# YukinoriMatsuoka/indy-plenum

Measured on AMD Instinct MI355X. Metric: Ed25519 verifies/sec at 1/8 MI355X (256B msgs) + % of INT32 VALU peak vs host CPU, higher is better.
Workload: dtype int32

## Files before the change

indy-plenum_amd/csrc/edv_hostcheck.cpp:

```cpp
#define EDV_CHAIN_FLOOR 1
#include <stdint.h>
#include <string.h>
#include <vector>
#include "edv_verify_core.h"
#include "edv_sha256.h"
#include "edv_merkle.h"
#include "edv_ledger.h"
#include "edv_tables.h"
#include "edv_hostplan.h"
#include "edv_selftest_cases.h"
#include "edv_probe_ops.h"

using namespace edv;

namespace {
struct HostATab {
  ge_cached t[kAEntries];
  int staged = 0;
  void store(int e, const ge_cached& c) { t[e] = c; }
  ge_cached load(int e) const { return t[e]; }
  void stage(int e) { staged = e; }
  ge_cached fetch() const { return t[staged]; }
};
struct HostBTab {
// ... 94 lines not shown
    const uint64_t mlen = off[i + 1] - off[i];
    std::vector<uint8_t> buf(mlen + 48, 0);
    if (mlen) memcpy(buf.data() + 16, msgs + off[i], mlen);
    uint32_t o[8];
    sha256_msg(o, buf.data() + 16, mlen);
    store_words(out + 32 * i, o, 8);
  }
  return 0;
}
int hc_btab_entries_of_bits(int bits, int t, const int32_t* js, int nj, int32_t* out) {
  if (bits != kBBits && bits != kBBitsCompact) return -1;
  const HostBTab& b = btab(bits);
  if (t < 0 || t >= b.sh.tables) return -1;
  for (int k = 0; k < nj; k++) {
    if (js[k] < 0 || js[k] >= b.sh.entries) return -1;
    btab_entry(out + size_t(k) * kBStride, js[k], b.base[t]);
  }
  return 0;
}
int hc_btab_entries_of(int t, const int32_t* js, int nj, int32_t* out) {
  return hc_btab_entries_of_bits(kBBits, t, js, nj, out);
}
int hc_rside_point_bits(int bits, const uint8_t* R32, const uint8_t* S32, uint8_t* out32) {
  struct Keep {
    ge_cached q;
    void store(int e, const ge_cached& c) { if (e == 1) q = c; }
  } tab;
  uint32_t R[8], S[8], o[8];
  load_words(R, R32, 8);
  load_words(S, S32, 8);
  if (bits != kBBits && bits != kBBitsCompact) return -1;
  HostBStage bs{btab(bits)};
  if (!prep_rpoint(R, S, tab, bs)) return -1;
  const fe two_y = fe_carry32(fe_add(tab.q.YpX, tab.q.YmX)), two_x = fe_carry32(fe_sub(tab.q.YpX, tab.q.YmX));
  ge_p2 p{two_x, two_y, fe_carry32(fe_add(tab.q.Z, tab.q.Z))};
  ge_p2_tobytes(o, p);
  store_words(out32, o, 8);
  return 0;
}
int hc_rside_point(const uint8_t* R32, const uint8_t* S32, uint8_t* out32) {
  return hc_rside_point_bits(kBBits, R32, S32, out32);
}
int hc_half_scalars(const uint8_t* h32, uint8_t* a32, uint8_t* u32) {
  uint32_t h[8], a[8], u[8];
  load_words(h, h32, 8);
  bool neg = false;
  half_scalars(h, a, u, neg);
  store_words(a32, a, 8);
  store_words(u32, u, 8);
  return neg ? 1 : 0;
}
int hc_probe_math(int op, const void* in, uint64_t in_stride, void* out, uint64_t out_stride, uint64_t n) {
  const ProbeSize sz = probe_size(op);
  if (!sz.in || probe_is_quad(op) || in_stride < sz.in || out_stride < sz.out || (in_stride & 3) || (out_stride & 3))
    return -1;
  for (uint64_t i = 0; i < n; i++) {
    const uint32_t* x = reinterpret_cast<const uint32_t*>(static_cast<const uint8_t*>(in) + i * in_stride);
    uint32_t* y = reinterpret_cast<uint32_t*>(static_cast<uint8_t*>(out) + i * out_stride);
    switch (op) {
#define HC_PROBE_CASE(OP) case OP: probe_lane_op<OP>(x, y); break;
      HC_PROBE_CASE(EDV_PROBE_FE_MUL)
      HC_PROBE_CASE(EDV_PROBE_FE_SQ)
      HC_PROBE_CASE(EDV_PROBE_FE_SQ2)
      HC_PROBE_CASE(EDV_PROBE_FE_SQ_FLOOR)
      HC_PROBE_CASE(EDV_PROBE_FE_TOBYTES)
      HC_PROBE_CASE(EDV_PROBE_FE_FROMBYTES)
      HC_PROBE_CASE(EDV_PROBE_FE_INVERT_SAFEGCD)
      HC_PROBE_CASE(EDV_PROBE_FE_POW22523)
      HC_PROBE_CASE(EDV_PROBE_SC_REDUCE)
      HC_PROBE_CASE(EDV_PROBE_HALF_SCALARS)
      HC_PROBE_CASE(EDV_PROBE_RECODE5)
      HC_PROBE_CASE(EDV_PROBE_APPROX_DIV)
      HC_PROBE_CASE(EDV_PROBE_FDIV_FLOOR)
      HC_PROBE_CASE(EDV_PROBE_EUCLID_DIV)
      HC_PROBE_CASE(EDV_PROBE_GE_FROMBYTES)
      HC_PROBE_CASE(EDV_PROBE_SC_MULADD)
      HC_PROBE_CASE(EDV_PROBE_RECODE8)
      HC_PROBE_CASE(EDV_PROBE_GE_P3_TOBYTES)
#undef HC_PROBE_CASE
      case EDV_PROBE_SCALARMULT_BASE: probe_scalarmult_base(x, y, comb()); break;
      default: return -1;
    }
  }
  return 0;
}
static_assert(kAEntries * 40 == 360, "a slot's table is 9 entries of 4 x 10 limbs");
int hc_stage_prep(const uint8_t* sigs, const uint8_t* pks, const uint8_t* msgs, const uint64_t* off, uint64_t n,
                  int bits, int side0, int nsides, int buckets, uint64_t cap, uint32_t* dig, uint8_t* alive,
                  int32_t* atab, int32_t* rtab, uint32_t* perm, uint8_t* accept) {
  if ((bits != kBBits && bits != kBBitsCompact) || n > cap || side0 < 0 || nsides < 1 || side0 + nsides > 3) return -1;
  const HostBTab& bt = btab(bits);
  if (buckets) {
    auto bucket = [&](uint64_t i) {
      const uint64_t nb = (64 + (off[i + 1] - off[i]) + 17 + 127) / 128;
      return nb < 63 ? nb : uint64_t(63);
    };
    uint64_t k = 0;
    bool one = true;
    for (uint64_t i = 1; i < n; i++) one = one && bucket(i) == bucket(0);
    for (uint64_t b = 0; b < 64 && !one; b++)
      for (uint64_t i = 0; i < n; i++)
        if (bucket(i) == b) perm[k++] = uint32_t(i);
    for (uint64_t i = 0; one && i < n; i++) perm[i] = uint32_t(i);
  }
  for (uint64_t j = 0; j < n; j++) {
    const uint64_t i = buckets ? perm[j] : j;
    uint32_t R[8], S[8], A[8];
    load_words(R, sigs + 64 * i, 8);
    load_words(S, sigs + 64 * i + 32, 8);
    load_words(A, pks + 32 * i, 8);
    for (int side = side0; side < side0 + nsides; side++) {
      bool ok;
      if (side == 0) {
        const uint64_t mlen = off[i + 1] - off[i];
        std::vector<uint8_t> buf(mlen + 32, 0);
        if (mlen) memcpy(buf.data() + 16, msgs + off[i], mlen);
        PrepDigits pd;
        ok = prep_one(R, S, A, buf.data() + 16, mlen, pd);
        if (ok) {
          for (int k = 0; k < 8; k++) {
            dig[uint64_t(k) * cap + j] = pd.da[k];
            dig[uint64_t(8 + k) * cap + j] = pd.db[k];
          }
          dig[16 * cap + j] = uint32_t(pd.nwin) | (pd.negR ? 0x100u : 0u);
        }
      } else {
        HostATab tab;
        if (side == 1) {
          ok = prep_point(A, tab);
        } else {
          HostBStage bs{bt};
          ok = prep_rpoint(R, S, tab, bs);
        }
        int32_t* o = (side == 1 ? atab : rtab) + j * 360;
        for (int e = 0; ok && e < kAEntries; e++) {
          from_fe(o + 40 * e, tab.t[e].YpX);
          from_fe(o + 40 * e + 10, tab.t[e].YmX);
          from_fe(o + 40 * e + 20, tab.t[e].Z);
          from_fe(o + 40 * e + 30, tab.t[e].T2d);
        }
      }
      alive[uint64_t(side) * cap + j] = ok ? 1 : 0;
      if (!ok) accept[i] = 0;
    }
  }
  return 0;
}
int hc_stage_main(uint64_t n, uint64_t cap, const uint32_t* dig, const uint8_t* alive, const int32_t* atab,
                  const int32_t* rtab, const uint32_t* perm, uint8_t* accept) {
  if (n > cap) return -1;
  auto live = [&](uint64_t j) { return j < n && alive[j] && alive[cap + j] && alive[2 * cap + j]; };
  for (uint64_t w0 = 0; w0 < n; w0 += 64) {
    int nwin = 0;
    for (uint64_t j = w0; j < w0 + 64; j++)
      if (live(j)) nwin = mx(nwin, int(dig[16 * cap + j] & 0xff));
    if (nwin > kAWindows) return -1;
    for (uint64_t j = w0; j < w0 + 64; j++) {
      if (!live(j)) continue;
      if (perm && perm[j] >= n) return -1;
      uint32_t da[8], db[8];
      for (int k = 0; k < 8; k++) {
        da[k] = dig[uint64_t(k) * cap + j];
        db[k] = dig[uint64_t(8 + k) * cap + j];
      }
      HostATab at, rt;
      for (int e = 0; e < kAEntries; e++) {
        const int32_t *a = atab + j * 360 + 40 * e, *r = rtab + j * 360 + 40 * e;
        at.t[e] = ge_cached{to_fe(a), to_fe(a + 10), to_fe(a + 20), to_fe(a + 30)};
        rt.t[e] = ge_cached{to_fe(r), to_fe(r + 10), to_fe(r + 20), to_fe(r + 30)};
      }
      accept[perm ? perm[j] : j] = main_one(da, db, nwin, (dig[16 * cap + j] >> 8) & 1, at, rt) ? 1 : 0;
    }
  }
  return 0;
}
namespace {
void put_p3(int32_t* pt, int k, uint64_t slots, uint64_t j, const ge_p3& p) {
  const fe* c[4] = {&p.X, &p.Y, &p.Z, &p.T};
  for (int q = 0; q < 4; q++)
    for (int i = 0; i < 10; i++) pt[(uint64_t(k) * 40 + 10 * q + i) * slots + j] = c[q]->v[i];
}
ge_p3 get_p3(const int32_t* pt, int k, uint64_t slots, uint64_t j) {
  fe c[4];
  for (int q = 0; q < 4; q++)
    for (int i = 0; i < 10; i++) c[q].v[i] = pt[(uint64_t(k) * 40 + 10 * q + i) * slots + j];
  return ge_p3{c[0], c[1], c[2], c[3]};
}
ge_p3 p3_add(const ge_p3& p, const ge_p3& q) { return ge_p1p1_to_p3(ge_add(p, ge_p3_to_cached(q))); }
ge_p3 p3_neg(const ge_p3& p) { return ge_p3{fe_neg(p.X), p.Y, p.Z, fe_neg(p.T)}; }
ge_p3 signed_digit_mult(const uint32_t d[8], bool negate, const ge_p3& P) {
  ge_p3 m[9];
  m[0] = ge_p3_identity();
  for (int e = 1; e < 9; e++) m[e] = p3_add(m[e - 1], P);
  ge_p3 acc = ge_p3_identity();
  for (int k = 63; k >= 0; k--) {
    for (int t = 0; t < 4; t++) acc = ge_p1p1_to_p3(ge_p2_dbl(ge_p3_to_p2(acc)));
    int dg = int(d[k / 8] >> (4 * (k % 8))) & 15;
    if (dg >= 8) dg -= 16;
    if (negate) dg = -dg;
    if (dg) acc = p3_add(acc, dg < 0 ? p3_neg(m[-dg]) : m[dg]);
  }
  return acc;
}
}
int hc_stage_latency_phase1(const uint8_t* sigs, const uint8_t* pks, const uint8_t* msgs, const uint64_t* off,
                            uint64_t n, int ns, int bits, uint32_t* dig, int32_t* pt, uint8_t* ok) {
  if ((bits != kBBits && bits != kBBitsCompact) || (ns != 16 && ns != 32) || n == 0) return -1;
  const HostBTab& bt = btab(bits);
  const uint64_t slots = (n + ns - 1) / ns * ns;
  for (uint64_t jl = 0; jl < slots; jl++) {
    const bool in = jl < n || jl < 16;
    const uint64_t i = jl < n ? jl : n - 1;
    bool ok0 = false, ok1 = false, ok2 = false;
    PrepDigits pd;
    ge_p3 pa = ge_p3_identity(), pr = ge_p3_identity(), sb = ge_p3_identity();
    if (in) {
      uint32_t R[8], S[8], A[8];
      load_words(R, sigs + 64 * i, 8);
      load_words(S, sigs + 64 * i + 32, 8);
      load_words(A, pks + 32 * i, 8);
      const uint64_t mlen = off[i + 1] - off[i];
      std::vector<uint8_t> buf(mlen + 32, 0);
      if (mlen) memcpy(buf.data() + 16, msgs + off[i], mlen);
      ok0 = prep_one(R, S, A, buf.data() + 16, mlen, pd);
      ok1 = ge_is_canonical(A) && !has_small_order(A) && ge_frombytes_negate(pa, A);
      if (!ok1) pa = ge_p3_identity();
      ok2 = ge_is_canonical(R) && !has_small_order(R) && ge_frombytes_negate(pr, R);
      if (!ok2) pr = ge_p3_identity();
      HostBStage bs{bt};
      add_sb(sb, S, bs);
    }
    for (int k = 0; k < 8; k++) {
      dig[uint64_t(k) * slots + jl] = ok0 ? pd.da[k] : 0u;
      dig[uint64_t(8 + k) * slots + jl] = ok0 ? pd.db[k] : 0u;
    }
    dig[16 * slots + jl] = ok0 ? (uint32_t(pd.nwin) | (pd.negR ? 0x100u : 0u)) : 0u;
    ok[jl] = ok0;
    ok[slots + jl] = ok1;
    ok[2 * slots + jl] = ok2;
    put_p3(pt, 0, slots, jl, pa);
    put_p3(pt, 1, slots, jl, pr);
    put_p3(pt, 2, slots, jl, sb);
  }
  return 0;
}
int hc_stage_latency_walk(uint64_t n, int ns, const uint32_t* dig, const int32_t* pt, const uint8_t* ok,
                          uint8_t* accept) {
  if ((ns != 16 && ns != 32) || n == 0) return -1;
  const uint64_t slots = (n + ns - 1) / ns * ns;
  for (uint64_t j = 0; j < n; j++) {
    const bool alive = ok[j] && ok[slots + j] && ok[2 * slots + j];
    if (!alive) {
      accept[j] = 0;
      continue;
    }
    const uint32_t wf = dig[16 * slots + j];
    if ((wf & 0xff) > uint32_t(kAWindows)) return -1;
    uint32_t da[8], db[8];
    for (int k = 0; k < 8; k++) {
      da[k] = dig[uint64_t(k) * slots + j];
      db[k] = dig[uint64_t(8 + k) * slots + j];
    }
    const ge_p3 q = p3_add(get_p3(pt, 2, slots, j), get_p3(pt, 1, slots, j));
    const ge_p3 r = p3_add(signed_digit_mult(da, false, get_p3(pt, 0, slots, j)),
                           signed_digit_mult(db, (wf >> 8) & 1, q));
    accept[j] = (fe_iszero(r.X) && fe_iszero(fe_sub(r.Y, r.Z))) ? 1 : 0;
  }
  return 0;
}
int hc_comb_entries(const int32_t* ij, int n, int32_t* out) {
  const HostComb& ct = comb();
  for (int k = 0; k < n; k++) {
    if (ij[2 * k] < 0 || ij[2 * k] >= kCombRows || ij[2 * k + 1] < 0 || ij[2 * k + 1] >= kCombEntries) return -1;
    memcpy(out + size_t(k) * kBStride, ct.w.data() + (ij[2 * k] * kCombEntries + ij[2 * k + 1]) * kBStride,
           kBStride * sizeof(int32_t));
  }
  return 0;
}
double hc_approx_div(double a, double b) { return approx_div(a, b); }
double hc_fdiv_floor(double a, double b) { return fdiv_floor(a, b); }
void hc_euclid_div(uint32_t* r0, uint32_t* t0, const uint32_t* r1, const uint32_t* t1) { euclid_div(r0, t0, r1, t1); }
int hc_recode5_windows(const uint8_t* in32, uint32_t* out8) {
  uint32_t w[8];
  load_words(w, in32, 8);
  recode5(out8, w);
  return digits5_windows(out8);
}
int hc_ge_frombytes_negate_limbs(const uint8_t* in32, int32_t* out40) {
  uint32_t w[8];
  load_words(w, in32, 8);
  ge_p3 p;
  const bool ok = ge_frombytes_negate(p, w);
  from_fe(out40, p.X);
  from_fe(out40 + 10, p.Y);
  from_fe(out40 + 20, p.Z);
  from_fe(out40 + 30, p.T);
  return int(ge_is_canonical(w)) | int(has_small_order(w)) << 1 | int(ok) << 2;
}
void hc_ge_add_p3(const int32_t* p40, const int32_t* q40, int32_t* out40) {
  const ge_p3 p{to_fe(p40), to_fe(p40 + 10), to_fe(p40 + 20), to_fe(p40 + 30)};
  const ge_p3 q{to_fe(q40), to_fe(q40 + 10), to_fe(q40 + 20), to_fe(q40 + 30)};
  const ge_p3 r = ge_p1p1_to_p3(ge_add(p, ge_p3_to_cached(q)));
  from_fe(out40, r.X); from_fe(out40 + 10, r.Y); from_fe(out40 + 20, r.Z); from_fe(out40 + 30, r.T);
}
void hc_ge_dbl_p3(const int32_t* p40, int32_t* out40) {
  const ge_p3 p{to_fe(p40), to_fe(p40 + 10), to_fe(p40 + 20), to_fe(p40 + 30)};
  const ge_p3 r = ge_p1p1_to_p3(ge_p2_dbl(ge_p3_to_p2(p)));
  from_fe(out40, r.X); from_fe(out40 + 10, r.Y); from_fe(out40 + 20, r.Z); from_fe(out40 + 30, r.T);
}
void hc_layout(int32_t* out4) {
  const int32_t v[4] = {kAWin, kAEntries, kBBits, kBTables};
  memcpy(out4, v, sizeof v);
}
int hc_btab_entries() { return kBEntries; }
void hc_ledger(int64_t n, const int64_t* failed, int nf, const int64_t* queries, int nq, int* out) {
  AsyncLedger l;
  for (int64_t i = 0; i < n; i++) l.issue();
  for (int k = 0; k < nf; k++) l.fail(failed[k]);
  for (int k = 0; k < nq; k++) out[k] = l.settled(queries[k]);
}
void hc_choose_tables(int policy, uint64_t n, int have_compact, int have_large, int failed, int* out3) {
  const TableChoice c = choose_tables(policy, n, have_compact != 0, have_large != 0, failed != 0);
  out3[0] = c.use;
  out3[1] = c.build;
  out3[2] = c.failed ? 1 : 0;
}
void hc_packed_layout(uint64_t n, uint64_t mbytes, uint64_t* out5) {
// ... 317 lines not shown
```

indy-plenum_amd/csrc/edv_verify.hip:

```cpp
#include <hip/hip_runtime.h>
#include <stdint.h>

#include "edv_verify_core.h"
#include "edv_kernels.h"
#include "edv_launch.h"
#include "edv_sha256.h"

using namespace edv;

namespace {

constexpr int kEntryPieces = 10;
constexpr int kLdsAWords = kEntryPieces * 256;
constexpr int kLdsWaveWords = 2 * kLdsAWords;
__device__ __forceinline__ void wait_staged() { asm volatile("s_waitcnt vmcnt(0)" ::: "memory"); }
struct LdsATab {
  const int32_t* slot;
  int32_t* lds;
  int lane;
  __device__ __forceinline__ void stage(int e) {
    const int32_t* g = slot + e * kEntryWords;
#pragma unroll
    for (int q = 0; q < kEntryPieces; q++)
      __builtin_amdgcn_global_load_lds(const_cast<int32_t*>(g + 4 * q), lds + q * 256, 16, 0, 0);
  }
  __device__ __forceinline__ ge_cached fetch() {
    wait_staged();
    int32_t t[4 * kEntryPieces];
#pragma unroll
    for (int q = 0; q < kEntryPieces; q++) {
      const int4 v = reinterpret_cast<const int4*>(lds + q * 256)[lane];
      t[4 * q] = v.x; t[4 * q + 1] = v.y; t[4 * q + 2] = v.z; t[4 * q + 3] = v.w;
    }
    ge_cached c;
#pragma unroll
    for (int l = 0; l < 10; l++) {
      c.YpX.v[l] = t[l]; c.YmX.v[l] = t[10 + l]; c.Z.v[l] = t[20 + l]; c.T2d.v[l] = t[30 + l];
    }
    return c;
  }
};
#define EDV_MAIN_BODY \
  const uint64_t j = uint64_t(blockIdx.x) * kBlock + threadIdx.x; \
  const bool live = j < a.n && a.st.alive[j] && a.st.alive[a.st.cap + j] && a.st.alive[2 * a.st.cap + j]; \
  const uint32_t* d = a.st.dig + j; \
  const uint64_t cap = a.st.cap; \
  const uint32_t wf = live ? d[uint64_t(kDigNwin) * cap] : 0; \
  int nwin = int(wf & 0xff); \
_Pragma("unroll") \
  for (int o = 32; o > 0; o >>= 1) nwin = max(nwin, __shfl_xor(nwin, o)); \
  nwin = __builtin_amdgcn_readfirstlane(nwin); \
  if (!live) return; \
  const uint64_t i = a.base + (a.st.perm ? a.st.perm[j] : j); \
  uint32_t da[8], db[8]; \
_Pragma("unroll") \
  for (int k = 0; k < 8; k++) { \
    da[k] = d[uint64_t(k) * cap]; \
    db[k] = d[uint64_t(8 + k) * cap]; \
  } \
_Pragma("unroll") \
  for (int k = 0; k < 8; k++) { \
    da[k] = uint32_t(opaque_i32(int32_t(da[k]))); \
    db[k] = uint32_t(opaque_i32(int32_t(db[k]))); \
  } \
  int32_t* wl = lds_main + (threadIdx.x >> 6) * kLdsWaveWords; \
  const int lane = int(threadIdx.x & 63); \
  LdsATab at{a.st.atab + j * kAWords, wl, lane}, rt{a.st.rtab + j * kAWords, wl + kLdsAWords, lane}; \
  a.accept[i] = main_one(da, db, nwin, (wf >> 8) & 1, at, rt) ? 1 : 0;

__global__ __launch_bounds__(kBlock) void edv_main_kernel(VerifyArgs a) {
  __shared__ int32_t lds_main[(kBlock / 64) * kLdsWaveWords];
  EDV_MAIN_BODY
}

constexpr int kSplitMainPrio = 2;
__global__ __launch_bounds__(kBlock) void edv_main_kernel_prio(VerifyArgs a) {
  __shared__ int32_t lds_main[(kBlock / 64) * kLdsWaveWords];
  __builtin_amdgcn_s_setprio(kSplitMainPrio);
  EDV_MAIN_BODY
}

__global__ __launch_bounds__(kBlock) void edv_sign_kernel(const uint32_t* seeds, const uint8_t* msgs,
                                                          const uint64_t* off, uint64_t msg_base, uint64_t n,
                                                          uint32_t* pks, uint32_t* sigs, const int32_t* comb) {
  const uint64_t i = uint64_t(blockIdx.x) * kBlock + threadIdx.x;
  if (i >= n) return;
  uint32_t seed[8], pk[8], sig[16];
  load_words(seed, seeds + 8 * i, 2);
  const uint64_t o0 = off[i] - msg_base, o1 = off[i + 1] - msg_base;
  sign_one(pk, sig, seed, msgs + o0, o1 - o0, GlobalComb{comb});
  uint4* po = reinterpret_cast<uint4*>(pks + 8 * i);
  uint4* so = reinterpret_cast<uint4*>(sigs + 16 * i);
  po[0] = make_uint4(pk[0], pk[1], pk[2], pk[3]);
  po[1] = make_uint4(pk[4], pk[5], pk[6], pk[7]);
#pragma unroll
  for (int k = 0; k < 4; k++) so[k] = make_uint4(sig[4 * k], sig[4 * k + 1], sig[4 * k + 2], sig[4 * k + 3]);
}

__global__ void edv_comb_kernel(int32_t* out) {
  const int t = threadIdx.x + blockIdx.x * blockDim.x;
  if (t < kCombRows * kCombEntries) comb_entry(out + t * kBStride, t / kCombEntries, t % kCombEntries);
}

__device__ __forceinline__ uint32_t sha_bucket(const uint64_t* off, uint64_t i) {
  const uint64_t nb = (64 + (off[i + 1] - off[i]) + 17 + 127) / 128;
  return nb < kBuckets - 1 ? uint32_t(nb) : uint32_t(kBuckets - 1);
}
__global__ __launch_bounds__(kBlock) void edv_bucket_hist_kernel(const uint64_t* off, uint64_t base, uint64_t n,
                                                                 uint32_t* hist) {
  __shared__ uint32_t h[kBuckets];
  if (threadIdx.x < kBuckets) h[threadIdx.x] = 0;
  __syncthreads();
  const uint64_t j = uint64_t(blockIdx.x) * kBlock + threadIdx.x;
  if (j < n) atomicAdd(&h[sha_bucket(off, base + j)], 1u);
  __syncthreads();
  if (threadIdx.x < kBuckets && h[threadIdx.x]) atomicAdd(&hist[threadIdx.x], h[threadIdx.x]);
}
__global__ __launch_bounds__(kBlock) void edv_bucket_scatter_kernel(const uint64_t* off, uint64_t base, uint64_t n,
                                                                    const uint32_t* hist, uint32_t* cursor,
                                                                    uint32_t* perm) {
  __shared__ uint32_t start[kBuckets], cnt[kBuckets], wbase[kBuckets];
  __shared__ int nonempty;
  if (threadIdx.x == 0) {
    uint32_t acc = 0;
    int ne = 0;
    for (int b = 0; b < kBuckets; b++) { start[b] = acc; acc += hist[b]; ne += hist[b] != 0; }
    nonempty = ne;
  }
  if (threadIdx.x < kBuckets) cnt[threadIdx.x] = 0;
  __syncthreads();
  const uint64_t j = uint64_t(blockIdx.x) * kBlock + threadIdx.x;
  if (nonempty <= 1) {
    if (j < n) perm[j] = uint32_t(j);
    return;
  }
  uint32_t b = 0, rank = 0;
  if (j < n) {
    b = sha_bucket(off, base + j);
    rank = atomicAdd(&cnt[b], 1u);
  }
  __syncthreads();
  if (threadIdx.x < kBuckets && cnt[threadIdx.x])
    wbase[threadIdx.x] = start[threadIdx.x] + atomicAdd(&cursor[threadIdx.x], cnt[threadIdx.x]);
  __syncthreads();
  if (j < n) perm[wbase[b] + rank] = uint32_t(j);
}

__global__ __launch_bounds__(kBlock) void edv_pack_bits_kernel(const uint8_t* acc, uint64_t n, uint8_t* bits) {
  const uint64_t k = uint64_t(blockIdx.x) * kBlock + threadIdx.x;
  if (8 * k >= n) return;
  uint32_t b = 0;
  if (8 * k + 8 <= n && !(reinterpret_cast<uintptr_t>(acc) & 3)) {
    const uint32_t lo = reinterpret_cast<const uint32_t*>(acc)[2 * k], hi = reinterpret_cast<const uint32_t*>(acc)[2 * k + 1];
#pragma unroll
    for (int t = 0; t < 4; t++) b |= (((lo >> (8 * t)) & 0xff) != 0 ? 1u : 0u) << t;
#pragma unroll
    for (int t = 0; t < 4; t++) b |= (((hi >> (8 * t)) & 0xff) != 0 ? 1u : 0u) << (4 + t);
  } else {
    for (uint64_t i = 8 * k; i < n && i < 8 * k + 8; i++) b |= (acc[i] != 0 ? 1u : 0u) << (i - 8 * k);
  }
  bits[k] = uint8_t(b);
}

__global__ void edv_bbase_kernel(ge_p3* bases, SbShape sh) {
  if (int(threadIdx.x) < sh.tables) bases[threadIdx.x] = base_point(int(threadIdx.x) * sh.bits);
}
__global__ void edv_btab_kernel(int32_t* out, const ge_p3* bases, SbShape sh) {
  const uint32_t t = threadIdx.x + blockIdx.x * blockDim.x;
  if (t < uint32_t(sh.tables * sh.entries))
    btab_entry(out + size_t(t) * kBStride, int(t % uint32_t(sh.entries)), bases[t / uint32_t(sh.entries)]);
}

__global__ __launch_bounds__(kBlock) void edv_sha256_kernel(const uint8_t* msgs, const uint64_t* off, uint64_t msg_base,
                                                            uint64_t n, uint32_t* out) {
  const uint64_t i = uint64_t(blockIdx.x) * kBlock + threadIdx.x;
  if (i >= n) return;
  const uint64_t o0 = off[i] - msg_base, o1 = off[i + 1] - msg_base;
  uint32_t d[8];
  sha256_msg(d, msgs + o0, o1 - o0);
  uint4* po = reinterpret_cast<uint4*>(out + 8 * i);
  po[0] = make_uint4(d[0], d[1], d[2], d[3]);
  po[1] = make_uint4(d[4], d[5], d[6], d[7]);
}

}

namespace edv {

hipError_t launch_main_kernel(unsigned blocks, hipStream_t s, const VerifyArgs& va, bool prio) {
  if (prio) edv_main_kernel_prio<<<dim3(blocks), dim3(kBlock), 0, s>>>(va);
  else edv_main_kernel<<<dim3(blocks), dim3(kBlock), 0, s>>>(va);
  return hipGetLastError();
}
hipError_t launch_bucket_kernels(unsigned blocks, hipStream_t s, const uint64_t* off, uint64_t base, uint64_t n,
                                 uint32_t* ctr, uint32_t* perm) {
  edv_bucket_hist_kernel<<<dim3(blocks), dim3(kBlock), 0, s>>>(off, base, n, ctr);
  edv_bucket_scatter_kernel<<<dim3(blocks), dim3(kBlock), 0, s>>>(off, base, n, ctr, ctr + kBuckets, perm);
  return hipGetLastError();
}
hipError_t launch_btab_kernel(hipStream_t s, int32_t* out, SbShape sh) {
  ge_p3* bases = reinterpret_cast<ge_p3*>(out + sb_words(sh));
  edv_bbase_kernel<<<1, 64, 0, s>>>(bases, sh);
  edv_btab_kernel<<<(sh.tables * sh.entries + 63) / 64, 64, 0, s>>>(out, bases, sh);
  return hipGetLastError();
}
hipError_t launch_comb_kernel(hipStream_t s, int32_t* out) {
  edv_comb_kernel<<<(kCombRows * kCombEntries + 63) / 64, 64, 0, s>>>(out);
  return hipGetLastError();
}
hipError_t launch_sign_kernel(unsigned blocks, hipStream_t s, const uint32_t* seeds, const uint8_t* msgs,
                              const uint64_t* off, uint64_t msg_base, uint64_t n, uint32_t* pks, uint32_t* sigs,
                              const int32_t* comb) {
  edv_sign_kernel<<<dim3(blocks), dim3(kBlock), 0, s>>>(seeds, msgs, off, msg_base, n, pks, sigs, comb);
  return hipGetLastError();
}
hipError_t launch_pack_bits_kernel(hipStream_t s, const uint8_t* acc, uint64_t n, uint8_t* bits) {
  const uint64_t nb = (n + 7) / 8;
  edv_pack_bits_kernel<<<dim3(unsigned((nb + kBlock - 1) / kBlock)), dim3(kBlock), 0, s>>>(acc, n, bits);
  return hipGetLastError();
}
hipError_t launch_sha256_kernel(unsigned blocks, hipStream_t s, const uint8_t* msgs, const uint64_t* off,
// ... 7 lines not shown
```

indy-plenum_amd/csrc/edv_verify_core.h:

```cpp
#pragma once
#include "edv_math.h"

namespace edv {

constexpr int kAWin = 4;
constexpr int kAWindows = (255 + kAWin - 1) / kAWin;
constexpr int kAEntries = (1 << (kAWin - 1)) + 1;
constexpr int kBBits = 22;
constexpr int kBTables = (253 + kBBits - 1) / kBBits;
constexpr int kBEntries = (1 << (kBBits - 1)) + 1;
constexpr int kBBitsCompact = 16;
constexpr int kBTablesCompact = (253 + kBBitsCompact - 1) / kBBitsCompact;
constexpr int kBEntriesCompact = (1 << (kBBitsCompact - 1)) + 1;
static_assert(253 - kBBits * (kBTables - 1) <= kBBits - 1, "top [S]B digit out of table range");
static_assert(253 - kBBitsCompact * (kBTablesCompact - 1) <= kBBitsCompact - 1, "top [S]B digit out of table range");
struct SbShape {
  int bits, tables, entries;
};
EDV_HD constexpr SbShape sb_large() { return SbShape{kBBits, kBTables, kBEntries}; }
EDV_HD constexpr SbShape sb_compact() { return SbShape{kBBitsCompact, kBTablesCompact, kBEntriesCompact}; }
constexpr int kCombEntries = 129;
constexpr int kBStride = 32;

EDV_HD int mx(int a, int b) { return a > b ? a : b; }
// ... 403 lines not shown
#pragma unroll
  for (int i = 0; i < 7; i++) v[i] = (v[i] >> N) | (v[i + 1] << (32 - N));
  v[7] >>= N;
}

EDV_HD ge_precomp precomp_from_words(const int32_t* w) {
  ge_precomp q;
#pragma unroll
  for (int l = 0; l < 10; l++) { q.ypx.v[l] = w[l]; q.ymx.v[l] = w[10 + l]; q.xy2d.v[l] = w[20 + l]; }
  return q;
}

EDV_HD ge_p3 base_point(int shift) {
  const uint32_t Bw[8] = {0x66666658u, 0x66666666u, 0x66666666u, 0x66666666u,
                          0x66666666u, 0x66666666u, 0x66666666u, 0x66666666u};
  ge_p3 nB;
  ge_frombytes_negate(nB, Bw);
  ge_p3 B{fe_neg(nB.X), nB.Y, nB.Z, fe_neg(nB.T)};
  for (int k = 0; k < shift; k++) B = ge_p1p1_to_p3(ge_p2_dbl(ge_p3_to_p2(B)));
  return B;
}
EDV_HD void btab_entry(int32_t* o, int j, const ge_p3& base) {
  const ge_cached Bc = ge_p3_to_cached(base);
  ge_p3 acc = ge_p3_identity();
  for (int bit = kBBits - 1; bit >= 0; bit--) {
    acc = ge_p1p1_to_p3(ge_p2_dbl(ge_p3_to_p2(acc)));
    if ((j >> bit) & 1) acc = ge_p1p1_to_p3(ge_add(acc, Bc));
  }
  const fe zi = fe_invert(acc.Z);
  const fe x = fe_mul(acc.X, zi), y = fe_mul(acc.Y, zi);
  const fe ypx = fe_carry32(fe_add(y, x)), ymx = fe_carry32(fe_sub(y, x));
  const fe xy2d = fe_mul(fe_mul(x, y), fe_d2());
  for (int l = 0; l < 10; l++) { o[l] = ypx.v[l]; o[10 + l] = ymx.v[l]; o[20 + l] = xy2d.v[l]; }
  o[30] = 0;
  o[31] = 0;
}

EDV_HD constexpr size_t sb_words(SbShape sh) { return size_t(sh.tables) * size_t(sh.entries) * kBStride; }
EDV_HD constexpr size_t sb_alloc_bytes(SbShape sh) { return 4 * sb_words(sh) + size_t(sh.tables) * sizeof(ge_p3); }

struct PrepDigits {
  uint32_t da[8];
  uint32_t db[8];
  int nwin;
  bool negR;
};

template <class Tab>
EDV_HD void build_table(Tab& tab, const ge_p3& P) {
  const ge_cached c1 = ge_p3_to_cached(P);
  const ge_precomp p1{c1.YpX, c1.YmX, c1.T2d};
  tab.store(0, ge_cached_identity());
  tab.store(1, c1);
  ge_p3 cur = ge_p1p1_to_p3(ge_p2_dbl(ge_p3_to_p2(P)));
  tab.store(2, ge_p3_to_cached(cur));
#pragma unroll 1
  for (int e = 3; e < kAEntries; e++) {
    cur = ge_p1p1_to_p3(ge_madd(cur, p1));
    tab.store(e, ge_p3_to_cached(cur));
  }
}
template <class Tab, class Stash>
EDV_HD void build_table_projective(Tab& tab, const ge_p3& P, Stash& st) {
  {
    const ge_cached c1 = ge_p3_to_cached(P);
    tab.store(0, ge_cached_identity());
    tab.store(1, c1);
    st.put(c1);
  }
  ge_p3 cur = ge_p1p1_to_p3(ge_p2_dbl(ge_p3_to_p2(P)));
  tab.store(2, ge_p3_to_cached(cur));
#pragma unroll 1
  for (int e = 3; e < kAEntries; e++) {
    cur = ge_p1p1_to_p3(ge_add(cur, st.get()));
    tab.store(e, ge_p3_to_cached(cur));
  }
}

EDV_HD bool prep_one(const uint32_t R[8], const uint32_t S[8], const uint32_t A[8], const uint8_t* m, uint64_t mlen,
                     PrepDigits& pd) {
  bool ok = !((S[7] & 0xF0000000u) && !sc_is_canonical(S));
  ok = ok && !has_small_order(R);
  ok = ok && ge_is_canonical(A) && !has_small_order(A);
  if (!ok) return false;
  uint32_t dig[16], h[8];
  hram(dig, R, A, m, mlen);
  sc_reduce(h, dig);
  uint32_t a[8], u[8];
  bool neg;
  half_scalars(h, a, u, neg);
  recode5(pd.da, a);
  recode5(pd.db, u);
  pd.nwin = mx(digits5_windows(pd.da), digits5_windows(pd.db));
  pd.negR = neg;
  return true;
}

template <class ATab>
EDV_HD bool prep_point(const uint32_t P[8], ATab& tab) {
  if (!ge_is_canonical(P) || has_small_order(P)) return false;
  ge_p3 nP;
  if (!ge_frombytes_negate(nP, P)) return false;
  build_table(tab, nP);
  return true;
}

EDV_HD void shr256_var(uint32_t v[8], int n) {
#pragma unroll
  for (int i = 0; i < 7; i++) v[i] = (v[i] >> n) | (v[i + 1] << (32 - n));
  v[7] >>= n;
}
template <class BTab>
EDV_HD void add_sb(ge_p3& q, const uint32_t S[8], BTab& bt) {
  const SbShape sh = bt.shape();
  uint32_t s[8];
#pragma unroll
  for (int i = 0; i < 8; i++) s[i] = S[i];
  s[7] &= 0x1fffffffu;
  int carry = 0;
  const int bits = sh.bits;
  auto next_digit = [&](bool top) {
    int e = int(s[0] & ((1u << bits) - 1)) + carry;
    shr256_var(s, bits);
    carry = top ? 0 : (e + (1 << (bits - 1))) >> bits;
    return e - carry * (1 << bits);
  };
  int dt = next_digit(sh.tables == 1);
  bt.stage(0, dt < 0 ? -dt : dt);
#pragma unroll 1
  for (int t = 0; t < sh.tables; t++) {
    const ge_precomp e = ge_precomp_cneg(bt.fetch(), dt < 0);
    if (t + 1 < sh.tables) {
      dt = next_digit(t + 2 == sh.tables);
      bt.stage(t + 1, dt < 0 ? -dt : dt);
    }
    q = ge_p1p1_to_p3(ge_madd(q, e));
  }
}
template <class BTab>
EDV_HD bool rpoint_q(const uint32_t R[8], const uint32_t S[8], BTab& bt, ge_p3& q) {
  if (!ge_is_canonical(R) || has_small_order(R)) return false;
  if (!ge_frombytes_negate(q, R)) return false;
  add_sb(q, S, bt);
  return true;
}
template <class ATab, class BTab>
EDV_HD bool prep_rpoint(const uint32_t R[8], const uint32_t S[8], ATab& tab, BTab& bt) {
  ge_p3 q;
  if (!rpoint_q(R, S, bt, q)) return false;
  build_table_projective(tab, q, bt);
  return true;
}

template <class ATab>
EDV_HD bool main_one(uint32_t da[8], uint32_t db[8], int nwin, bool negR, ATab& at, ATab& rt) {
  constexpr int kTop = kAWin * (kAWindows - 1);
  constexpr int kTopShl = 32 - kAWin - (kTop - 224);
#pragma unroll 1
  for (int k = nwin; k < kAWindows; k++) {
    shl256<kAWin>(da);
    shl256<kAWin>(db);
  }
  ge_p2 acc = ge_p2_identity();
#pragma unroll 1
  for (int w = nwin - 1; w >= 0; --w) {
    const int dA = int32_t(da[7] << kTopShl) >> (32 - kAWin);
    const int dR = int32_t(db[7] << kTopShl) >> (32 - kAWin);
    shl256<kAWin>(da);
    shl256<kAWin>(db);
    at.stage(dA < 0 ? -dA : dA);
    rt.stage(dR < 0 ? -dR : dR);
    ge_p3 p3;
    if (w == nwin - 1) {
      p3 = ge_p3_identity();
    } else {
#pragma unroll 1
      for (int d = 0; d < kAWin - 1; d++) acc = ge_p1p1_to_p2(ge_p2_dbl(acc));
      p3 = ge_p1p1_to_p3(ge_p2_dbl(acc));
    }
    const ge_cached ea = at.fetch();
    p3 = ge_p1p1_to_p3(ge_add(p3, ge_cached_cneg(ea, dA < 0)));
    const ge_cached er = rt.fetch();
    acc = ge_p1p1_to_p2(ge_add(p3, ge_cached_cneg(er, (dR < 0) != negR)));
  }
  return fe_iszero(acc.X) && fe_iszero(fe_carry32(fe_sub(acc.Y, acc.Z)));
}

template <class ATab, class BTab>
EDV_HD bool verify_one(const uint32_t R[8], const uint32_t S[8], const uint32_t A[8], const uint8_t* m, uint64_t mlen,
                       ATab& at, ATab& rt, BTab& bt) {
  PrepDigits pd;
  if (!prep_one(R, S, A, m, mlen, pd)) return false;
  if (!prep_point(A, at) || !prep_rpoint(R, S, rt, bt)) return false;
  return main_one(pd.da, pd.db, pd.nwin, pd.negR, at, rt);
}

constexpr int kCombRows = 32;
EDV_HD void comb_entry(int32_t* o, int i, int j) {
  const uint32_t Bw[8] = {0x66666658u, 0x66666666u, 0x66666666u, 0x66666666u,
                          0x66666666u, 0x66666666u, 0x66666666u, 0x66666666u};
  ge_p3 nB;
  ge_frombytes_negate(nB, Bw);
  ge_p3 base{fe_neg(nB.X), nB.Y, nB.Z, fe_neg(nB.T)};
  for (int k = 0; k < 8 * i; k++) base = ge_p1p1_to_p3(ge_p2_dbl(ge_p3_to_p2(base)));
  const ge_cached bc = ge_p3_to_cached(base);
  ge_p3 acc = ge_p3_identity();
  for (int bit = 7; bit >= 0; bit--) {
    acc = ge_p1p1_to_p3(ge_p2_dbl(ge_p3_to_p2(acc)));
    if ((j >> bit) & 1) acc = ge_p1p1_to_p3(ge_add(acc, bc));
  }
  const fe zi = fe_invert(acc.Z);
  const fe x = fe_mul(acc.X, zi), y = fe_mul(acc.Y, zi);
  const fe ypx = fe_carry32(fe_add(y, x)), ymx = fe_carry32(fe_sub(y, x));
  const fe xy2d = fe_mul(fe_mul(x, y), fe_d2());
  for (int l = 0; l < 10; l++) { o[l] = ypx.v[l]; o[10 + l] = ymx.v[l]; o[20 + l] = xy2d.v[l]; }
  o[30] = 0;
  o[31] = 0;
}
template <class CombTab>
EDV_HD ge_p3 scalarmult_base(const uint32_t k[8], const CombTab& ct) {
  uint32_t d[8];
  recode8(d, k);
  ge_p3 acc = ge_p3_identity();
#pragma unroll 1
  for (int i = 0; i < kCombRows; i++) {
    const int di = int(int8_t(uint8_t(d[i >> 2] >> (8 * (i & 3)))));
    const int ui = di < 0 ? -di : di;
    acc = ge_p1p1_to_p3(ge_madd(acc, ge_precomp_cneg(ct.entry(i, ui), di < 0)));
  }
  return acc;
}
EDV_HD void ge_p3_tobytes(uint32_t w[8], const ge_p3& p) { ge_p2_tobytes(w, ge_p3_to_p2(p)); }

EDV_HD void sc_muladd(uint32_t out[8], const uint32_t a[8], const uint32_t b[8], const uint32_t c[8]) {
  uint32_t t[16];
  uint64_t carry = 0;
#pragma unroll
  for (int k = 0; k < 16; k++) {
    uint64_t lo = carry + (k < 8 ? c[k] : 0), hi = 0;
#pragma unroll
    for (int i = 0; i < 8; i++) {
      const int j = k - i;
      if (j < 0 || j > 7) continue;
      const uint64_t p = uint64_t(a[i]) * b[j];
      const uint64_t s = lo + p;
      hi += (s < lo);
      lo = s;
    }
    t[k] = uint32_t(lo);
    carry = (lo >> 32) | (hi << 32);
  }
  sc_reduce(out, t);
}

template <class CombTab>
EDV_HD void sign_one(uint32_t pk[8], uint32_t sig[16], const uint32_t seed[8], const uint8_t* m, uint64_t mlen,
                     const CombTab& ct) {
  uint32_t az[16];
  sha512_pm<32>(az, seed, m, 0);
  az[0] &= ~7u;
  az[7] = (az[7] & 0x7fffffffu) | 0x40000000u;
  uint32_t a64[16], a[8];
#pragma unroll
  for (int k = 0; k < 16; k++) a64[k] = k < 8 ? az[k] : 0;
  sc_reduce(a, a64);
  ge_p3_tobytes(pk, scalarmult_base(a, ct));
  uint32_t nonce[16], r[8];
  sha512_pm<32>(nonce, az + 8, m, mlen);
  sc_reduce(r, nonce);
  ge_p3_tobytes(sig, scalarmult_base(r, ct));
  uint32_t hr[16], h[8];
  hram(hr, sig, pk, m, mlen);
  sc_reduce(h, hr);
  uint32_t aclamped[8];
#pragma unroll
  for (int k = 0; k < 8; k++) aclamped[k] = az[k];
  sc_muladd(sig + 8, h, aclamped, r);
}

}
```

Measured before the change: 97.80 million.

## Fold small top window digit into table-entry additions to skip four doublings

When the wave's top window index is 34 and every lane's top digit is small (0..2), the top window is folded away. It is replaced by up to two additions of table entry 8 (which equals 8P) before the next window, so 16·e·P is handled as 2·(e·8P). That removes one window's four doublings at the cost of up to four extra point additions and wave-wide ballots. Host check paths and test helpers are extended to mirror the new recoding.

After: 97.98 million (median of 6 runs). No clear change (+0.2%).

```diff
diff --git a/indy-plenum_amd/csrc/edv_hostcheck.cpp b/indy-plenum_amd/csrc/edv_hostcheck.cpp
--- a/indy-plenum_amd/csrc/edv_hostcheck.cpp
+++ b/indy-plenum_amd/csrc/edv_hostcheck.cpp
@@ -270,9 +270,16 @@
   auto live = [&](uint64_t j) { return j < n && alive[j] && alive[cap + j] && alive[2 * cap + j]; };
   for (uint64_t w0 = 0; w0 < n; w0 += 64) {
     int nwin = 0;
-    for (uint64_t j = w0; j < w0 + 64; j++)
-      if (live(j)) nwin = mx(nwin, int(dig[16 * cap + j] & 0xff));
+    uint32_t max_e = 0;
+    for (uint64_t j = w0; j < w0 + 64; j++) {
+      if (!live(j)) continue;
+      const uint32_t ea = (dig[uint64_t(kWideWord) * cap + j] >> kWideShift) & 15u;
+      const uint32_t eb = (dig[uint64_t(8 + kWideWord) * cap + j] >> kWideShift) & 15u;
+      nwin = mx(nwin, wide_fold_count(int(dig[16 * cap + j] & 0xff), ea, eb));
+      max_e = (ea | eb) & 2u ? 2u : (max_e ? max_e : ((ea | eb) ? 1u : 0u));
+    }
     if (nwin > kAWindows) return -1;
+    const int wide = wide_rounds(nwin, max_e);
     for (uint64_t j = w0; j < w0 + 64; j++) {
       if (!live(j)) continue;
       if (perm && perm[j] >= n) return -1;
@@ -287,10 +294,62 @@
         at.t[e] = ge_cached{to_fe(a), to_fe(a + 10), to_fe(a + 20), to_fe(a + 30)};
         rt.t[e] = ge_cached{to_fe(r), to_fe(r + 10), to_fe(r + 20), to_fe(r + 30)};
       }
-      accept[perm ? perm[j] : j] = main_one(da, db, nwin, (dig[16 * cap + j] >> 8) & 1, at, rt) ? 1 : 0;
+      accept[perm ? perm[j] : j] =
+          main_one(da, db, nwin, (dig[16 * cap + j] >> 8) & 1, at, rt, wide, wide_digit(da), wide_digit(db)) ? 1 : 0;
     }
   }
   return 0;
+}
+void hc_wide_recode(const uint8_t* in32, uint32_t* out8, int32_t* out3) {
+  uint32_t w[8];
+  load_words(w, in32, 8);
+  recode5(out8, w);
+  const int own = digits5_windows(out8);
+  const uint32_t e = wide_digit(out8);
+  const int nwin = wide_fold_count(own, e, 0);
+  out3[0] = nwin;
+  out3[1] = own;
+  out3[2] = nwin < own ? int32_t(e) : 0;
+  if (nwin < own) out8[kWideWord] &= ~(15u << kWideShift);
+}
+void hc_wide_lane(const uint8_t* a32, const uint8_t* u32, int32_t* out4) {
+  uint32_t a[8], u[8], da[8], db[8];
+  load_words(a, a32, 8);
+  load_words(u, u32, 8);
+  recode5(da, a);
+  recode5(db, u);
+  const int own = mx(digits5_windows(da), digits5_windows(db));
+  const int nwin = wide_fold_count(own, wide_digit(da), wide_digit(db));
+  out4[0] = own;
+  out4[1] = nwin;
+  out4[2] = nwin < own ? int32_t(wide_digit(da)) : 0;
+  out4[3] = nwin < own ? int32_t(wide_digit(db)) : 0;
+}
+int hc_main_one(const uint8_t* a32, const uint8_t* u32, int negR, const int32_t* p1_40, const int32_t* p2_40,
+                int wave_nwin, int wide) {
+  uint32_t a[8], u[8], da[8], db[8];
+  load_words(a, a32, 8);
+  load_words(u, u32, 8);
+  recode5(da, a);
+  recode5(db, u);
+  const uint32_t ea = wide_digit(da), eb = wide_digit(db);
+  const int own = wide_fold_count(mx(digits5_windows(da), digits5_windows(db)), ea, eb);
+  const int nwin = wave_nwin ? wave_nwin : own;
+  const uint32_t me = ea > eb ? ea : eb;
+  if (nwin < own || nwin > kAWindows) return -1;
+  if (wide < 0) wide = wide_rounds(nwin, me);
+  if (wide < wide_rounds(nwin, me) || (wide && (nwin != kWideWin || wide > int(kWideMaxE)))) return -1;
+  HostATab at, rt;
+  const ge_p3 p1{to_fe(p1_40), to_fe(p1_40 + 10), to_fe(p1_40 + 20), to_fe(p1_40 + 30)};
+  const ge_p3 p2{to_fe(p2_40), to_fe(p2_40 + 10), to_fe(p2_40 + 20), to_fe(p2_40 + 30)};
+  struct NoStash {
+    ge_cached c;
+    void put(const ge_cached& x) { c = x; }
+    ge_cached get() const { return c; }
+  } st;
+  build_table_projective(at, p1, st);
+  build_table_projective(rt, p2, st);
+  return main_one(da, db, nwin, negR != 0, at, rt, wide, ea, eb) ? 1 : 0;
 }
 namespace {
 void put_p3(int32_t* pt, int k, uint64_t slots, uint64_t j, const ge_p3& p) {
diff --git a/indy-plenum_amd/csrc/edv_verify.hip b/indy-plenum_amd/csrc/edv_verify.hip
--- a/indy-plenum_amd/csrc/edv_verify.hip
+++ b/indy-plenum_amd/csrc/edv_verify.hip
@@ -46,10 +46,13 @@
   const uint32_t* d = a.st.dig + j; \
   const uint64_t cap = a.st.cap; \
   const uint32_t wf = live ? d[uint64_t(kDigNwin) * cap] : 0; \
-  int nwin = int(wf & 0xff); \
+  const uint32_t ea = live ? (d[uint64_t(kWideWord) * cap] >> kWideShift) & 15u : 0; \
+  const uint32_t eb = live ? (d[uint64_t(8 + kWideWord) * cap] >> kWideShift) & 15u : 0; \
+  int nwin = wide_fold_count(int(wf & 0xff), ea, eb); \
 _Pragma("unroll") \
   for (int o = 32; o > 0; o >>= 1) nwin = max(nwin, __shfl_xor(nwin, o)); \
   nwin = __builtin_amdgcn_readfirstlane(nwin); \
+  const int wide = wide_rounds(nwin, __ballot(((ea | eb) & 2u) != 0) ? 2u : (__ballot((ea | eb) != 0) ? 1u : 0u)); \
   if (!live) return; \
   const uint64_t i = a.base + (a.st.perm ? a.st.perm[j] : j); \
   uint32_t da[8], db[8]; \
@@ -66,7 +69,7 @@
   int32_t* wl = lds_main + (threadIdx.x >> 6) * kLdsWaveWords; \
   const int lane = int(threadIdx.x & 63); \
   LdsATab at{a.st.atab + j * kAWords, wl, lane}, rt{a.st.rtab + j * kAWords, wl + kLdsAWords, lane}; \
-  a.accept[i] = main_one(da, db, nwin, (wf >> 8) & 1, at, rt) ? 1 : 0;
+  a.accept[i] = main_one(da, db, nwin, (wf >> 8) & 1, at, rt, wide, ea, eb) ? 1 : 0;
 
 __global__ __launch_bounds__(kBlock) void edv_main_kernel(VerifyArgs a) {
   __shared__ int32_t lds_main[(kBlock / 64) * kLdsWaveWords];
diff --git a/indy-plenum_amd/csrc/edv_verify_core.h b/indy-plenum_amd/csrc/edv_verify_core.h
--- a/indy-plenum_amd/csrc/edv_verify_core.h
+++ b/indy-plenum_amd/csrc/edv_verify_core.h
@@ -579,16 +579,61 @@
   return true;
 }
 
+constexpr int kWideWin = 33;
+constexpr uint32_t kWideMaxE = 2;
+static_assert(kAWin == 4, "the wide top is laid out for 4-bit windows: 16 e P = 2 (e x entry 8)");
+constexpr int kWideWord = (4 * kWideWin) >> 5, kWideShift = (4 * kWideWin) & 31;
+EDV_HD uint32_t wide_digit(const uint32_t d[8]) { return (d[kWideWord] >> kWideShift) & 15u; }
+EDV_HD int wide_fold_count(int nwin, uint32_t ea, uint32_t eb) {
+  static_assert(kWideMaxE == 2, "the range test below is e + 1 < 4");
+  const uint32_t out = nz_mask(uint32_t(nwin) ^ uint32_t(kWideWin + 1)) | nz_mask(((ea + 1) | (eb + 1)) >> 2);
+  return nwin - int(~out & 1u);
+}
+EDV_HD int wide_rounds(int wave_nwin, uint32_t max_e) { return wave_nwin == kWideWin ? int(max_e) : 0; }
+
 template <class ATab>
-EDV_HD bool main_one(uint32_t da[8], uint32_t db[8], int nwin, bool negR, ATab& at, ATab& rt) {
+EDV_HD bool main_one(uint32_t da[8], uint32_t db[8], int nwin, bool negR, ATab& at, ATab& rt, int wide = 0,
+                     uint32_t ea = 0, uint32_t eb = 0) {
   constexpr int kTop = kAWin * (kAWindows - 1);
   constexpr int kTopShl = 32 - kAWin - (kTop - 224);
+  if (wide) {
+    at.stage(int((((ea + 1) >> 1) & 1u) << 3));
+    rt.stage(int((((eb + 1) >> 1) & 1u) << 3));
+  }
 #pragma unroll 1
   for (int k = nwin; k < kAWindows; k++) {
     shl256<kAWin>(da);
     shl256<kAWin>(db);
   }
   ge_p2 acc = ge_p2_identity();
+  int top = nwin - 1;
+  if (wide) {
+    ge_p3 s = ge_p3_identity();
+#pragma unroll 1
+    for (int r = 0; r < wide; r++) {
+      if (r) {
+        at.stage(int((((ea + 1 - uint32_t(r)) >> 1) & 1u) << 3));
+        rt.stage(int((((eb + 1 - uint32_t(r)) >> 1) & 1u) << 3));
+      }
+      const ge_cached ca = at.fetch();
+      s = ge_p1p1_to_p3(ge_add(s, ca));
+      const ge_cached cr = rt.fetch();
+      s = ge_p1p1_to_p3(ge_add(s, ge_cached_cneg(cr, negR)));
+    }
+    const int dA = int32_t(da[7] << kTopShl) >> (32 - kAWin);
+    const int dR = int32_t(db[7] << kTopShl) >> (32 - kAWin);
+    shl256<kAWin>(da);
+    shl256<kAWin>(db);
+    at.stage(dA < 0 ? -dA : dA);
+    rt.stage(dR < 0 ? -dR : dR);
+    s = ge_p1p1_to_p3(ge_p2_dbl(ge_p3_to_p2(s)));
+    const ge_cached ta = at.fetch();
+    s = ge_p1p1_to_p3(ge_add(s, ge_cached_cneg(ta, dA < 0)));
+    const ge_cached tr = rt.fetch();
+    acc = ge_p1p1_to_p2(ge_add(s, ge_cached_cneg(tr, (dR < 0) != negR)));
+    top = -1;
+    nwin -= 1;
+  }
 #pragma unroll 1
   for (int w = nwin - 1; w >= 0; --w) {
     const int dA = int32_t(da[7] << kTopShl) >> (32 - kAWin);
@@ -598,7 +643,7 @@
     at.stage(dA < 0 ? -dA : dA);
     rt.stage(dR < 0 ? -dR : dR);
     ge_p3 p3;
-    if (w == nwin - 1) {
+    if (w == top) {
       p3 = ge_p3_identity();
     } else {
 #pragma unroll 1
@@ -619,7 +664,9 @@
   PrepDigits pd;
   if (!prep_one(R, S, A, m, mlen, pd)) return false;
   if (!prep_point(A, at) || !prep_rpoint(R, S, rt, bt)) return false;
-  return main_one(pd.da, pd.db, pd.nwin, pd.negR, at, rt);
+  const uint32_t ea = wide_digit(pd.da), eb = wide_digit(pd.db);
+  const int nwin = wide_fold_count(pd.nwin, ea, eb);
+  return main_one(pd.da, pd.db, nwin, pd.negR, at, rt, wide_rounds(nwin, ea > eb ? ea : eb), ea, eb);
 }
 
 constexpr int kCombRows = 32;
```
